# alexkeroro86/SampleNeRFRO

Hardware: AMD Instinct MI355X
Metric: rays/sec (train step) (higher is better)
Workload: dtype f16x3/fp32-acc

## Files before the change

include/rnerf.h:

```cpp
#ifndef RNERF_H_
#define RNERF_H_

#include <stddef.h>
#include <stdint.h>

#ifdef __cplusplus
extern "C" {
#endif

#define RNERF_VERSION 4

enum rnerf_status {
  RNERF_OK = 0,
  RNERF_ERR_ARG = -1,
  RNERF_ERR_HIP = -2,
  RNERF_ERR_UNSUPPORTED = -3
};

enum rnerf_precision {
  RNERF_PREC_F32 = 0,
  RNERF_PREC_F16X3 = 1,
  RNERF_PREC_BF16X3 = 2,
  RNERF_PREC_F16 = 3,
  RNERF_PREC_BF16 = 4,
// ... 178 lines not shown
  int32_t bg_patch_size;
  double bg_weight, bg_smooth_weight, annealed_alpha;
  double frozen_sq;
  int64_t frozen_count;
  void* aux_stream;
  void* grads_stream;
} rnerf_train_cfg;
typedef struct rnerf_prefetch {
  const float* origins;
  const float* viewdirs;
  float* path_pd;
  float* path_dr;
  void* side_stream;
} rnerf_prefetch;
size_t rnerf_train_workspace_bytes(const rnerf_model* m, const rnerf_train_cfg* c, int32_t B);
int rnerf_train_forward_backward(const rnerf_model* m, const rnerf_train_cfg* c, const float* theta, const float* origins, const float* viewdirs,
                                 const float* pixels, const float* env_dirs, int32_t B, const uint32_t* keys4, const int32_t* jitter_override,
                                 const float* u_override, int32_t u_per_ray, const float* path_pd, const float* path_dr, float* grads,
                                 void* workspace, int32_t max_workgroups, const rnerf_prefetch* next, void* stream);

#define RNERF_ADAM_SCRATCH_FLOATS 3076
typedef struct rnerf_adam_cfg {
  double lr_init, lr_final, lr_delay_mult;
  int64_t max_steps, lr_delay_steps;
  double b1, b2, eps;
  double weight_decay_mult, grad_max_val, grad_max_norm;
  int64_t n_all;
  double lr_override;
  int32_t use_lr_override;
  int32_t skip_nonfinite;
} rnerf_adam_cfg;
int rnerf_adam_update(const rnerf_adam_cfg* c, float* theta, float* mu, float* nu, float* grads, int64_t n_theta, const float* frozen_params,
                      int64_t n_frozen, int32_t* step_counter, float* scratch, void* stream);

int rnerf_graph_begin(void* stream);
int rnerf_graph_end(void* stream, void** graph_exec);
int rnerf_graph_launch(void* graph_exec, void* stream);
int rnerf_graph_destroy(void* graph_exec);
int rnerf_fork(void* main_stream, void* side_stream);
int rnerf_join(void* main_stream, void* side_stream);

size_t rnerf_ssim_workspace_bytes(int64_t n, int32_t H, int32_t W, int32_t C, int32_t filter_size);
int rnerf_ssim(const float* img0, const float* img1, int64_t n, int32_t H, int32_t W, int32_t C, int32_t filter_size, double filter_sigma,
               double max_val, double k1, double k2, float* map, float* mean, void* workspace, void* stream);

#ifdef __cplusplus
}
#endif
#endif
```

samplenerfro_amd/_lib.py:

```python
from __future__ import annotations

import ctypes as C
import os
from typing import Optional

HERE = os.path.dirname(os.path.abspath(__file__))
LIB_PATH = os.path.join(HERE, "lib", "librnerf.so")

PREC_F32, PREC_F16X3, PREC_BF16X3, PREC_F16, PREC_BF16, PREC_F16X2, PREC_F16F8 = 0, 1, 2, 3, 4, 5, 6
PRECISIONS = {"f32": PREC_F32, "f16x3": PREC_F16X3, "bf16x3": PREC_BF16X3, "f16": PREC_F16, "bf16": PREC_BF16, "f16x2": PREC_F16X2, "f16f8": PREC_F16F8}
BWD_BF16, BWD_F16, BWD_F16X2 = 0, 1, 2
BWD_F16X3 = BWD_F16X2
BWD_F16X3_LO8 = 4
BACKWARDS = {"f16x3": BWD_F16X3, "f16x3lo8": BWD_F16X3_LO8, "f16": BWD_F16, "bf16": BWD_BF16, "f32": BWD_F16X3, "tf32": BWD_F16}
BACKWARD_NAMES = {BWD_F16X3: "f16x3", BWD_F16X3_LO8: "f16x3lo8", BWD_F16: "f16", BWD_BF16: "bf16"}
TWO_PLANE_BACKWARDS = (BWD_F16X3, BWD_F16X3_LO8)
ABI_VERSION = 4
NERFMLP_PARAMS = 595844
BKGDMLP_PARAMS = 56963
SO3MLP_PARAMS = 65411


class RnerfError(RuntimeError):
    pass
# ... 75 lines not shown
    "rnerf_nerfmlp_wgrad": (C.c_int, [C.c_int, C.c_int, _vp, _vp, _i64, _vp, _vp, _vp]),
    "rnerf_voxelize": (C.c_int, [_vp, _vp, _vp, _vp, _i32, _vp, _GP, _i32, _dbl, _dbl, _vp, _vp, _vp, _vp]),
    "rnerf_voxelize_samples": (C.c_int, [_vp, _vp, _vp, _vp, _i32, _vp, _GP, _i32, _vp, _vp, _vp]),
    "rnerf_voxelize_majority": (C.c_int, [_vp, _vp, _vp, _i32, _i32, _dbl, _dbl, _vp, _vp, _vp]),
    "rnerf_so3_query": (C.c_int, [_vp, _GP, _vp, _vp, _vp, _vp, _i64, _vp, _vp, _vp]),
    "rnerf_march_all": (C.c_int, [_vp, _GP, _vp, _vp, _vp, _vp, _vp, _i32, _dbl, _dbl, _i32, _vp, _vp, _vp, _vp, _vp]),
    "rnerf_generate_rays": (C.c_int, [_vp, _i32, _dbl, _dbl, _dbl, _dbl, _dbl, _i32, _i32, _i32, _vp, _vp, _vp, _vp]),
    "rnerf_sample_batch": (C.c_int, [_vp, _i32, _i32, _dbl, _dbl, _dbl, _dbl, _dbl, _i32, _i32, _vp, _i32, _vp, _i32, _vp, _vp, _vp, _vp, _vp, _vp]),
    "rnerf_stratified_u": (C.c_int, [_vp, _i32, _i32, _vp, _vp]),
    "rnerf_bkgd_save_bytes": (C.c_size_t, [_i64]),
    "rnerf_bkgd_dy_bytes": (C.c_size_t, [_i64]),
    "rnerf_bkgd_forward_train": (C.c_int, [_vp, _vp, _i32, _i64, _dbl, _vp, _vp, _vp]),
    "rnerf_bkgd_backward": (C.c_int, [_vp, _vp, _vp, _i64, _dbl, _vp, _vp, _vp, _vp]),
    "rnerf_theta_sumsq": (C.c_int, [_vp, _i64, _vp, _vp]),
    "rnerf_march_all_train": (C.c_int, [_vp, _GP, _vp, _vp, _vp, _vp, _vp, _i32, _dbl, _dbl, _i32, _vp, _vp, _vp, _vp, _i32, _vp, _vp, _vp, _vp, _vp, _vp]),
    "rnerf_so3_packed_bytes": (C.c_size_t, []),
    "rnerf_so3_save_bytes": (C.c_size_t, [_i64]),
    "rnerf_so3_dy_bytes": (C.c_size_t, [_i64]),
    "rnerf_so3_forward_train": (C.c_int, [_vp, _vp, _vp, _i64, _vp, _vp]),
    "rnerf_so3_backward": (C.c_int, [_vp, _vp, _vp, _vp, _i64, _vp, _i64, _vp, _vp, _vp, _vp]),
    "rnerf_so3_pair_jacobian": (C.c_int, [_vp, _GP, _vp, _vp, _vp, _vp, _i64, _vp, _vp, _vp]),
    "rnerf_march_adjoint": (C.c_int, [_vp, _GP, _vp, _vp, _vp, _vp, _vp, _vp, _vp, _vp, _i32, _dbl, _dbl, _i32, _vp, _vp]),
    "rnerf_nerfmlp_input_grad": (C.c_int, [_vp, C.c_int, _vp, _vp, _vp, _vp, _i32, _i32, _vp, _vp, _vp]),
    "rnerf_resample": (C.c_int, [_vp, _vp, _i32, _i32, _vp, _i32, _vp, _vp, _i32, _i32, _vp, _vp, _vp, _vp, _vp]),
    "rnerf_integrated_pos_enc": (C.c_int, [_vp, _vp, _vp, _i32, _i32, _vp, _dbl, _i32, _i32, _vp, _vp, _vp, _vp]),
    "rnerf_rng_split3": (C.c_int, [_vp, _vp, _vp]),
    "rnerf_rng_forward": (C.c_int, [_vp, _i32, _i32, _i32, _vp, _vp, _vp]),
    "rnerf_stratified_u_dev": (C.c_int, [_vp, _i32, _i32, _vp, _vp]),
    "rnerf_forward_workspace_bytes": (C.c_size_t, [_MP, _i32]),
    "rnerf_forward": (C.c_int, [_MP, _vp, _vp, _i32, _vp, _vp, _i32, _vp, _vp, _vp, _vp, _vp, _i32, _vp]),
    "rnerf_train_workspace_bytes": (C.c_size_t, [_MP, _TP, _i32]),
    "rnerf_train_forward_backward": (C.c_int, [_MP, _TP, _vp, _vp, _vp, _vp, _vp, _i32, _vp, _vp, _vp, _i32, _vp, _vp, _vp, _vp, _i32, C.POINTER(Prefetch), _vp]),
    "rnerf_adam_update": (C.c_int, [_AP, _vp, _vp, _vp, _vp, _i64, _vp, _i64, _vp, _vp, _vp]),
    "rnerf_graph_begin": (C.c_int, [_vp]),
    "rnerf_graph_end": (C.c_int, [_vp, C.POINTER(C.c_void_p)]),
    "rnerf_graph_launch": (C.c_int, [_vp, _vp]),
    "rnerf_graph_destroy": (C.c_int, [_vp]),
    "rnerf_fork": (C.c_int, [_vp, _vp]),
    "rnerf_join": (C.c_int, [_vp, _vp]),
    "rnerf_ssim_workspace_bytes": (C.c_size_t, [_i64, _i32, _i32, _i32, _i32]),
    "rnerf_ssim": (C.c_int, [_vp, _vp, _i64, _i32, _i32, _i32, _i32, _dbl, _dbl, _dbl, _dbl, _vp, _vp, _vp, _vp]),
}

_lib: Optional[C.CDLL] = None


def load(path: Optional[str] = None) -> C.CDLL:
    global _lib
    if _lib is not None and path is None:
        return _lib
    p = path or LIB_PATH
    if not os.path.exists(p):
        raise RnerfError(f"{p} not found: build it with `python -m samplenerfro_amd.build` "
                         "(there is no CPU fallback for the hot path)")
    lib = C.CDLL(p)
    for name, (res, args) in SIGNATURES.items():
        fn = getattr(lib, name)
        fn.restype = res
        fn.argtypes = args
    got = lib.rnerf_version()
    if got != ABI_VERSION:
        raise RnerfError(f"{p} speaks ABI version {got}, this binding was written for {ABI_VERSION} (include/rnerf.h RNERF_VERSION): rebuild with "
                         "`python -m samplenerfro_amd.build --force`")
    if path is None or _lib is None:
        _lib = lib
    return lib
# ... 18 lines not shown
```

samplenerfro_amd/csrc/pipeline.hip:

```cpp
#include "common.h"

#include <math.h>
#include <mutex>
#include <utility>
#include <vector>

namespace rnerf {
static int current_device_cus() {
  static int cache[64] = {0};
  int dev = 0;
  if (hipGetDevice(&dev) != hipSuccess || dev < 0 || dev >= 64) return 256;
  if (cache[dev] == 0) {
    int cus = 0;
    cache[dev] = (hipDeviceGetAttribute(&cus, hipDeviceAttributeMultiprocessorCount, dev) == hipSuccess && cus > 0) ? cus : 256;
  }
  return cache[dev];
}

namespace {
constexpr size_t kPoolCap = 32;
struct EventPool { std::vector<hipEvent_t> free_[64]; };
thread_local EventPool tl_pool;
inline hipError_t pool_get(hipEvent_t* e) {
  int dev = 0;
// ... 94 lines not shown
    u[(size_t)f * B + b] = fminf(fadd(fmul((float)f, s), r), one_m_eps);
  };
  put(j, x0);
  if (j + half < size) put(j + half, x1);
}

__global__ void linspace_u_kernel(int F, double stop, float* __restrict__ u) {
  const int i = blockIdx.x * blockDim.x + threadIdx.x;
  if (i >= F) return;
  const double step = F > 1 ? stop / (double)(F - 1) : 0.0;
  u[i] = (F > 1 && i == F - 1) ? (float)stop : (float)((double)i * step);
}

__global__ void __launch_bounds__(256) bkgd_dirs_kernel(const float4* __restrict__ path_dr, const int* __restrict__ jitter, int Nc, int B,
                                                        const float* __restrict__ env, int M, float4* __restrict__ dst) {
  const int i = blockIdx.x * blockDim.x + threadIdx.x;
  if (i < B) {
    const float4 d = path_dr[(size_t)jitter[Nc - 1] * B + i];
    dst[i] = make_float4(d.x, d.y, d.z, 0.f);
  } else if (i < B + M) {
    const int e = i - B;
    dst[i] = make_float4(env[3 * e], env[3 * e + 1], env[3 * e + 2], 0.f);
  }
}

__global__ void __launch_bounds__(256) bd_cut_mul_kernel(const float* __restrict__ trans, const float* __restrict__ behind, int B,
                                                         float* __restrict__ out) {
  const int i = blockIdx.x * blockDim.x + threadIdx.x;
  if (i < 3 * B) out[i] = fmul(trans[i / 3], behind[i]);
}

constexpr int ADAM_BLOCKS = 1024;
__global__ void __launch_bounds__(256) adam_prep_kernel(const float* __restrict__ theta, float* __restrict__ g, long long n, float wd2, float max_val,
                                                        int want_norm, float* __restrict__ partial, float* __restrict__ bad_partial) {
  float s = 0.f;
  int bad = 0;
  for (long long i = (long long)blockIdx.x * blockDim.x + threadIdx.x; i < n; i += (long long)gridDim.x * blockDim.x) {
    float v = g[i];
    if (wd2 != 0.f) v = v + theta[i] * wd2;
    const bool nf = !(fabsf(v) <= 3.402823466e38f);
    bad += nf;
    if (max_val > 0.f && !nf) v = fminf(fmaxf(v, -max_val), max_val);
    g[i] = v;
    s += v * v;
  }
  __shared__ float red[4];
  __shared__ int redb[4];
  for (int o = 32; o > 0; o >>= 1) { s += __shfl_down(s, o); bad += __shfl_down(bad, o); }
  if ((threadIdx.x & 63) == 0) { red[threadIdx.x >> 6] = s; redb[threadIdx.x >> 6] = bad; }
  __syncthreads();
  if (threadIdx.x == 0) {
    if (want_norm) partial[blockIdx.x] = (red[0] + red[1]) + (red[2] + red[3]);
    bad_partial[blockIdx.x] = (float)((redb[0] + redb[1]) + (redb[2] + redb[3]));
  }
}
__global__ void __launch_bounds__(256) adam_frozen_sq_kernel(const float* __restrict__ frozen, long long n, float wd2, float max_val,
                                                             float* __restrict__ partial) {
  float s = 0.f;
  for (long long i = (long long)blockIdx.x * blockDim.x + threadIdx.x; i < n; i += (long long)gridDim.x * blockDim.x) {
    float v = frozen[i] * wd2;
    if (max_val > 0.f) v = fminf(fmaxf(v, -max_val), max_val);
    s += v * v;
  }
  __shared__ float red[4];
  for (int o = 32; o > 0; o >>= 1) s += __shfl_down(s, o);
  if ((threadIdx.x & 63) == 0) red[threadIdx.x >> 6] = s;
  __syncthreads();
  if (threadIdx.x == 0) partial[blockIdx.x] = (red[0] + red[1]) + (red[2] + red[3]);
}
struct AdamSched { double lr_init, lr_final, lr_delay_mult, max_steps, lr_delay_steps, b1, b2, max_norm, lr_override; int use_override, skip_nonfinite; };
__global__ void __launch_bounds__(256) adam_scalars_kernel(AdamSched c, int* __restrict__ step, const float* __restrict__ partial, int n_partial,
                                                           const float* __restrict__ bad_partial, float* __restrict__ scal) {
  __shared__ double red[256];
  double s = 0.0;
  for (int i = threadIdx.x; i < n_partial; i += 256) s += (double)partial[i];
  red[threadIdx.x] = s;
  __syncthreads();
  for (int o = 128; o > 0; o >>= 1) { if ((int)threadIdx.x < o) red[threadIdx.x] += red[threadIdx.x + o]; __syncthreads(); }
  const double sumsq = red[0];
  __syncthreads();
  double nb = 0.0;
  if (bad_partial) for (int i = threadIdx.x; i < ADAM_BLOCKS; i += 256) nb += (double)bad_partial[i];
  red[threadIdx.x] = nb;
  __syncthreads();
  for (int o = 128; o > 0; o >>= 1) { if ((int)threadIdx.x < o) red[threadIdx.x] += red[threadIdx.x + o]; __syncthreads(); }
  if (threadIdx.x != 0) return;
  const int count = *step;
  const double t = (double)count + 1.0;
  double lr;
  if (c.use_override) {
    lr = c.lr_override;
  } else {
    double delay = 1.0;
    if (c.lr_delay_steps > 0) {
      const double x = fmin(fmax((double)count / c.lr_delay_steps, 0.0), 1.0);
      delay = c.lr_delay_mult + (1.0 - c.lr_delay_mult) * sin(0.5 * 3.141592653589793 * x);
    }
    const double start = fmin(fmax((double)count, 0.0), 1.0);
    const double tt = fmin(fmax(fmax((double)count, 0.0) / c.max_steps, 0.0), 1.0);
    lr = start * delay * exp(log(c.lr_init) * (1.0 - tt) + log(c.lr_final) * tt);
  }
  const double bad = red[0];
  scal[0] = (float)(-lr / (1.0 - pow(c.b1, t)));
  scal[1] = (c.skip_nonfinite && bad > 0.0) ? -1.0f : (float)(1.0 / (1.0 - pow(c.b2, t)));
  float mult = 1.0f;
  if (c.max_norm > 0) {
    const float norm = sqrtf((float)sumsq);
    mult = fminf((float)c.max_norm / (1e-7f + norm), 1.0f);
  }
  scal[2] = mult;
  scal[3] = (float)bad;
  *step = count + 1;
}
__global__ void __launch_bounds__(256) adam_apply_kernel(float* __restrict__ theta, float* __restrict__ mu, float* __restrict__ nu,
                                                         const float* __restrict__ g, long long n, float b1, float b2, float eps,
                                                         float* __restrict__ scal, int count_bad) {
  const float a = scal[0], c2 = scal[1], mult = scal[2];
  if (c2 < 0.f) return;
  int bad = 0;
  for (long long i = (long long)blockIdx.x * blockDim.x + threadIdx.x; i < n; i += (long long)gridDim.x * blockDim.x) {
    const float gi = g[i] * mult;
    bad += !(fabsf(gi) <= 3.402823466e38f);
    const float m = mu[i] * b1 + gi * (1.0f - b1);
    const float v = nu[i] * b2 + (gi * gi) * (1.0f - b2);
    mu[i] = m; nu[i] = v;
    theta[i] = theta[i] + a * (m / (sqrtf(v * c2) + eps));
  }
  if (count_bad && __builtin_amdgcn_ballot_w64(bad != 0) != 0) {
    for (int o = 32; o > 0; o >>= 1) bad += __shfl_down(bad, o);
    if ((threadIdx.x & 63) == 0 && bad) atomicAdd(&scal[3], (float)bad);
  }
}

struct Carver {
  char* base; size_t off;
  explicit Carver(void* b) : base((char*)b), off(0) {}
  template <typename T> T* take(size_t count) {
    off = (off + 255) & ~(size_t)255;
    T* p = (T*)(base ? base + off : nullptr);
    off += count * sizeof(T);
    return p;
  }
  void* bytes(size_t n) { return (void*)take<char>(n); }
};

struct FwdBuffers {
  float *path_pd, *path_dr, *bk_dirs, *bkgd, *raw_c, *weights, *u, *rows_pd, *rows_dr, *scratch, *raw_f, *tmp_level, *tmp_level2;
};
static size_t carve_forward(const rnerf_model* m, int32_t B, bool own_path, void* ws, FwdBuffers* f) {
  Carver c(ws);
  const size_t Nc = m->num_coarse, Nf = m->num_fine, N = Nc * (size_t)m->num_path, S = Nc + Nf;
  f->path_pd = own_path ? c.take<float>(N * B * 4) : nullptr;
  f->path_dr = own_path ? c.take<float>(N * B * 4) : nullptr;
  f->bk_dirs = c.take<float>((size_t)B * 4);
  f->bkgd = c.take<float>((size_t)B * 3);
  f->raw_c = c.take<float>(Nc * B * 4);
  f->weights = c.take<float>(Nc * B);
  f->u = f->rows_pd = f->rows_dr = f->scratch = f->raw_f = f->tmp_level = f->tmp_level2 = nullptr;
  if (Nf > 0) {
    f->u = c.take<float>(Nf * (size_t)B);
    f->rows_pd = c.take<float>(S * B * 4);
    f->rows_dr = c.take<float>(S * B * 4);
    f->scratch = c.take<float>(S * B);
// ... 300 lines not shown
  float* d_first = t.d_all;
  const bool split_levels = levels_side_by_side(m, c, B);
  float* d_raw_c = split_levels ? t.d_raw_c : t.d_raw;
  void* dy_c = split_levels ? t.dy_c : t.dy;
  if (Nf > 0) {
    RNERF_TRY(rnerf_composite_backward(f.raw_f, f.rows_pd, f.rows_dr, nullptr, S, B, bkgd, m->rgb_padding, m->sigma_bias, lf.rgb, pixels, lf.trans, lf.tb, t.sums,
                                       mse_scale, c->bg_weight * bg_on, t.d_raw, d_first, 0, m->white_bkgd, m->bd_cut == 1 ? 1 : level_mask_mode(m), m->bd_cut ? m->bd_cut_bbox : nullptr, stream));
    if (split_levels) {
      RNERF_TRY(rnerf_composite_backward(f.raw_c, path_pd, path_dr, jitter, Nc, B, bkgd, m->rgb_padding, m->sigma_bias, lc.rgb, pixels, nullptr, nullptr, nullptr,
                                         mse_scale, 0.0, d_raw_c, d_first, 1, m->white_bkgd, level_mask_mode(m), level_mask_box(m), stream));
      RNERF_TRY(rnerf_fork(stream, aux));
      if (smooth) RNERF_TRY(rnerf_env_smooth_backward(rgb_env, ps, c->bg_smooth_weight * env_on, t.d_all + (size_t)3 * B, t.env_sum, aux));
      RNERF_TRY(rnerf_bkgd_backward(th_b, t.save_bk, t.d_all, (int64_t)B + M, m->rgb_padding, t.dy_bk, g_b, nullptr, aux));
      RNERF_TRY(nerfmlp_dgrad_impl(t.packed_bwd, t.packed_c, prec, bwd, t.save_c, d_raw_c, (int64_t)Nc * B, dy_c, !pre_zeroed, false, (hipStream_t)aux));
      RNERF_TRY(rnerf_nerfmlp_wgrad(prec, bwd, t.save_c, dy_c, (int64_t)Nc * B, g_c, t.wgrad_ws_c, aux));
    }
    if (!aux) RNERF_TRY(rnerf_nerfmlp_pack_bwd(th_f, bwd, t.packed_bwd_f, stream));
    RNERF_TRY(nerfmlp_dgrad_impl(t.packed_bwd_f, t.packed_f, prec, bwd, t.save_f, t.d_raw, (int64_t)S * B, t.dy, !pre_zeroed, !split_levels, st));
    if (next) RNERF_TRY(march_next());
    RNERF_TRY(rnerf_nerfmlp_wgrad(prec, bwd, t.save_f, t.dy, (int64_t)S * B, g_f, t.wgrad_ws, stream));
    if (split_levels)
      RNERF_TRY(rnerf_join(stream, aux));
    else
      RNERF_TRY(rnerf_composite_backward(f.raw_c, path_pd, path_dr, jitter, Nc, B, bkgd, m->rgb_padding, m->sigma_bias, lc.rgb, pixels, nullptr, nullptr, nullptr,
                                         mse_scale, 0.0, t.d_raw, d_first, 1, m->white_bkgd, level_mask_mode(m), level_mask_box(m), stream));
  } else {
    RNERF_TRY(rnerf_composite_backward(f.raw_c, path_pd, path_dr, jitter, Nc, B, bkgd, m->rgb_padding, m->sigma_bias, lf.rgb, pixels, lf.trans, lf.tb, t.sums,
                                       mse_scale, c->bg_weight * bg_on, t.d_raw, d_first, 0, m->white_bkgd, level_mask_mode(m), level_mask_box(m), stream));
  }
  if (!aux) RNERF_TRY(rnerf_nerfmlp_pack_bwd(th_c, bwd, t.packed_bwd, stream));
  if (!split_levels)
    RNERF_TRY(nerfmlp_dgrad_impl(t.packed_bwd, t.packed_c, prec, bwd, t.save_c, t.d_raw, (int64_t)Nc * B, t.dy, !(pre_zeroed && Nf == 0), true, st));
  if (next && Nf == 0) RNERF_TRY(march_next());
  if (!split_levels) RNERF_TRY(rnerf_nerfmlp_wgrad(prec, bwd, t.save_c, t.dy, (int64_t)Nc * B, g_c, t.wgrad_ws, stream));
  if (c->grads_stream) RNERF_TRY(rnerf_fork(stream, c->grads_stream));
  if (!split_levels) {
    if (smooth) RNERF_TRY(rnerf_env_smooth_backward(rgb_env, ps, c->bg_smooth_weight * env_on, t.d_all + (size_t)3 * B, t.env_sum, stream));
    RNERF_TRY(rnerf_bkgd_backward(th_b, t.save_bk, t.d_all, (int64_t)B + M, m->rgb_padding, t.dy_bk, g_b, nullptr, stream));
  }
  RNERF_TRY(rnerf_train_stats(t.sums, B, Nf > 0, c->bg_weight * bg_on, smooth ? t.env_sum : nullptr, ps, env_on, aux ? nullptr : theta, n_theta, c->frozen_sq,
                              n_theta + c->frozen_count, stats8, stream));
  return RNERF_OK;
}

extern "C" int rnerf_adam_update(const rnerf_adam_cfg* c, float* theta, float* mu, float* nu, float* grads, int64_t n_theta, const float* frozen_params,
                                 int64_t n_frozen, int32_t* step_counter, float* scratch, void* stream) {
  RNERF_CHECK_ARG(c && theta && mu && nu && grads && step_counter && scratch, "rnerf_adam_update: null pointer");
  RNERF_CHECK_ARG(n_theta >= 1 && c->n_all >= n_theta, "rnerf_adam_update: need n_theta >= 1 and n_all >= n_theta");
  hipStream_t st = (hipStream_t)stream;
  const double wd2 = c->weight_decay_mult > 0 ? 2.0 * c->weight_decay_mult / (double)c->n_all : 0.0;
  const int want_norm = c->grad_max_norm > 0;
  float* scal = scratch;
  float* partial = scratch + 4;
  float* bad_partial = nullptr;
  int n_partial = 0;
  if (wd2 != 0.0 || c->grad_max_val > 0 || want_norm || c->skip_nonfinite) {
    bad_partial = scratch + 4 + 2 * ADAM_BLOCKS;
    hipLaunchKernelGGL(adam_prep_kernel, dim3(ADAM_BLOCKS), dim3(256), 0, st, (const float*)theta, grads, (long long)n_theta, (float)wd2, (float)c->grad_max_val,
                       want_norm, partial, bad_partial);
    if (want_norm) {
      n_partial = ADAM_BLOCKS;
      if (frozen_params && n_frozen > 0 && wd2 != 0.0) {
        hipLaunchKernelGGL(adam_frozen_sq_kernel, dim3(ADAM_BLOCKS), dim3(256), 0, st, frozen_params, (long long)n_frozen, (float)wd2, (float)c->grad_max_val,
                           partial + ADAM_BLOCKS);
        n_partial = 2 * ADAM_BLOCKS;
      }
    }
  }
  AdamSched s{c->lr_init, c->lr_final, c->lr_delay_mult, (double)c->max_steps, (double)c->lr_delay_steps, c->b1, c->b2, c->grad_max_norm, c->lr_override, c->use_lr_override != 0,
              c->skip_nonfinite != 0};
  hipLaunchKernelGGL(adam_scalars_kernel, dim3(1), dim3(256), 0, st, s, step_counter, (const float*)partial, n_partial, (const float*)bad_partial, scal);
  hipLaunchKernelGGL(adam_apply_kernel, dim3(ADAM_BLOCKS), dim3(256), 0, st, theta, mu, nu, (const float*)grads, (long long)n_theta, (float)c->b1, (float)c->b2,
                     (float)c->eps, scal, bad_partial == nullptr);
  RNERF_CHECK_LAUNCH();
  return RNERF_OK;
}

namespace {
std::mutex g_ev_mu;
thread_local std::vector<hipEvent_t> tl_capture_events;
std::vector<std::pair<void*, std::vector<hipEvent_t>>> g_graph_events;
void drop_events(std::vector<hipEvent_t>& v) {
  for (hipEvent_t e : v) (void)hipEventDestroy(e);
  v.clear();
}
}

extern "C" int rnerf_graph_begin(void* stream) {
  drop_events(tl_capture_events);
  RNERF_CHECK_HIP(hipStreamBeginCapture((hipStream_t)stream, hipStreamCaptureModeThreadLocal));
  return RNERF_OK;
}

extern "C" int rnerf_graph_end(void* stream, void** graph_exec) {
  RNERF_CHECK_ARG(graph_exec, "rnerf_graph_end: null pointer");
  hipGraph_t g = nullptr;
  hipError_t err = hipStreamEndCapture((hipStream_t)stream, &g);
  if (err != hipSuccess) { drop_events(tl_capture_events); set_error("hipStreamEndCapture failed: %s", hipGetErrorString(err)); return RNERF_ERR_HIP; }
  hipGraphExec_t e = nullptr;
  err = hipGraphInstantiate(&e, g, nullptr, nullptr, 0);
  hipGraphDestroy(g);
  if (err != hipSuccess) { drop_events(tl_capture_events); set_error("hipGraphInstantiate failed: %s", hipGetErrorString(err)); return RNERF_ERR_HIP; }
  {
    std::lock_guard<std::mutex> l(g_ev_mu);
    g_graph_events.emplace_back((void*)e, std::move(tl_capture_events));
  }
  tl_capture_events.clear();
  *graph_exec = (void*)e;
// ... 60 lines not shown
```

samplenerfro_amd/graph.py:

```python
from __future__ import annotations

import ctypes as C
import os
from typing import Any, Dict, Optional

import numpy as np
import torch

from . import _lib, distributed, ops
from .train import TrainState, _bump, adam_cfg, frozen_sq_of, train_cfg
from .utils import Rays, Stats


class GraphTrainStep:
    def __init__(self, model, state: TrainState, flags, batch_size: int, rng, env_rays: Optional[Rays] = None, annealed_alpha: float = 0.5,
                 prefetch: bool = True):
        if not flags.stage.startswith("radiance"):
            raise NotImplementedError("GraphTrainStep: the radiance stages (stage all* reads a device counter back every step)")
        if state._lr_fn_default is not state.lr_fn:
            raise ValueError("GraphTrainStep evaluates the reference's learning-rate schedule on the device; state.lr_fn was replaced")
        self.lib = _lib.load()
        self.model, self.state, self.flags = model, state, flags
        self.B = int(batch_size)
        dev = state.theta.device
# ... 59 lines not shown
        k = 1 - self.slot if self.prefetch else self.slot
        return {"origins": self.origins[k], "viewdirs": self.viewdirs[k], "pixels": self.pixels[k]}

    def order_after_loader(self) -> None:
        self.main.wait_stream(torch.cuda.current_stream())

    def _march(self, slot: int, stream) -> None:
        k = slot if self.prefetch else 0
        m = self.model
        _lib.check(self.lib.rnerf_march(m.table.data_ptr(), C.byref(m.spec), self.origins[slot].data_ptr(), self.viewdirs[slot].data_ptr(), self.B,
                                        m.near, m.far, m.num_samples, self.path_pd[k].data_ptr(), self.path_dr[k].data_ptr(), None, None, stream),
                   "rnerf_march")

    def _issue_front(self, slot: int) -> None:
        lib, st, sd = self.lib, self.main.cuda_stream, self.side.cuda_stream
        k = slot if self.prefetch else 0
        _lib.check(lib.rnerf_rng_split3(self.rng_state.data_ptr(), self.keys4.data_ptr(), st), "rnerf_rng_split3")
        if not self.prefetch:
            self._march(slot, st)
        nxt = None
        if self.prefetch:
            nxt = _lib.Prefetch(self.origins[1 - slot].data_ptr(), self.viewdirs[1 - slot].data_ptr(), self.path_pd[1 - slot].data_ptr(),
                                self.path_dr[1 - slot].data_ptr(), sd)
        _lib.check(lib.rnerf_train_forward_backward(C.byref(self.m), C.byref(self.c), self.state.theta.data_ptr(), self.origins[slot].data_ptr(),
                                                    self.viewdirs[slot].data_ptr(), self.pixels[slot].data_ptr(), _lib.ptr(self.env), self.B,
                                                    self.keys4.data_ptr(), None, None, 0, self.path_pd[k].data_ptr(), self.path_dr[k].data_ptr(),
                                                    self.state.grads.data_ptr(), self.ws.data_ptr(), 0, C.byref(nxt) if nxt is not None else None, st),
                   "rnerf_train_forward_backward")

    def _issue_back(self) -> None:
        s = self.state
        fs = frozen_sq_of(s, s.variables)
        frozen = s.variables["flat"].get("so3_mlp") if fs[1] > 0 else None
        _lib.check(self.lib.rnerf_adam_update(C.byref(self.a), s.theta.data_ptr(), s.mu.data_ptr(), s.nu.data_ptr(), s.grads.data_ptr(), s.theta.numel(),
                                              _lib.ptr(frozen), fs[1], s.step_dev.data_ptr(), s.adam_scratch.data_ptr(), self.main.cuda_stream),
                   "rnerf_adam_update")

    def _capture(self, slot: int):
        lib, st, sd = self.lib, self.main.cuda_stream, self.side.cuda_stream
        out = C.c_void_p()
        if not self.split:
            _lib.check(lib.rnerf_graph_begin(st), "rnerf_graph_begin")
            self._issue_front(slot)
            self._issue_back()
            if self.prefetch:
                _lib.check(lib.rnerf_join(st, sd), "rnerf_join")
            _lib.check(lib.rnerf_graph_end(st, C.byref(out)), "rnerf_graph_end")
            return (out.value, None)
        _lib.check(lib.rnerf_graph_begin(st), "rnerf_graph_begin")
        self._issue_front(slot)
        if self.prefetch:
            _lib.check(lib.rnerf_join(st, sd), "rnerf_join")
        _lib.check(lib.rnerf_graph_end(st, C.byref(out)), "rnerf_graph_end")
        back = C.c_void_p()
        _lib.check(lib.rnerf_graph_begin(st), "rnerf_graph_begin")
        self._issue_back()
        _lib.check(lib.rnerf_graph_end(st, C.byref(back)), "rnerf_graph_end")
        return (out.value, back.value)

    def _warm(self, slot: int) -> None:
        self._issue_front(slot)
        if self.prefetch:
            _lib.check(self.lib.rnerf_join(self.main.cuda_stream, self.side.cuda_stream), "rnerf_join")
        if self.split:
            with torch.cuda.stream(self.main):
                distributed.allreduce_mean_([self.state.grads])
        self._issue_back()

    def step(self, annealed_alpha: Optional[float] = None) -> Stats:
# ... 58 lines not shown
```

samplenerfro_amd/train.py:

```python
from __future__ import annotations

import contextlib
import ctypes as C
import os
import weakref
from typing import Any, Dict, Optional

import numpy as np
import torch

from . import _lib, distributed, ops, prng
from .models import BKGD_MLP_SHAPES, NERF_MLP_SHAPES, SO3_MLP_SHAPES, NerfModel, make_variables
from .utils import Rays, Stats, learning_rate_decay

_RANGE_RETRY_LAG = 2
_LAG_SLOTS = 8
_SKIP_NONFINITE_UPDATES = True

_N_STATS = 8


class TrainState:

    def __init__(self, step, theta, mu, nu, variables, segments, lr_fn, flags=None):
        self.step, self.theta, self.mu, self.nu = step, theta, mu, nu
        self.flags = flags
        self.variables, self.segments, self.lr_fn = variables, segments, lr_fn
        self.grads = torch.zeros(theta.numel() + _N_STATS, dtype=torch.float32, device=theta.device)
        self.frozen_sq: Optional[torch.Tensor] = None
        self.next_path = None
        self._lr_fn_default = lr_fn
        self.step_dev = torch.zeros(1, dtype=torch.int32, device=theta.device) if theta.is_cuda else None
        self._step_dev_value = 0
        self.adam_scratch = torch.zeros(_lib.ADAM_SCRATCH_FLOATS, dtype=torch.float32, device=theta.device) if theta.is_cuda else None
        self._staged_bad: Optional[int] = None
        self.range_retries = 0
        self.range_retry_failures = 0
        self._model_ref = None
        self._lag_pending = []
        self._lag_host = torch.zeros(_LAG_SLOTS, dtype=torch.float32).pin_memory() if theta.is_cuda else None
        self._lag_count = 0
        self.last_retry_stats = None

    def nonfinite_grads(self) -> int:
        if self._staged_bad is not None:
            return self._staged_bad
        return int(self.adam_scratch[3].item()) if self.adam_scratch is not None else 0

    def sync_step_counter(self) -> None:
        if self.step_dev is not None and self._step_dev_value != self.step:
            self.step_dev.fill_(int(self.step))
            self._step_dev_value = self.step

    @classmethod
    def create(cls, model: NerfModel, variables: Dict[str, Any], flags) -> "TrainState":
        names = ["coarse_mlp"] + (["fine_mlp"] if model.num_fine_samples > 0 else []) + ["bkgd_mlp"]
        stage = getattr(flags, "stage", "radiance")
        if stage.startswith("all"):
            names.append("so3_mlp")
        elif stage.startswith("ior"):
            names = ["so3_mlp"]
        shapes = {"coarse_mlp": NERF_MLP_SHAPES, "fine_mlp": NERF_MLP_SHAPES, "bkgd_mlp": BKGD_MLP_SHAPES, "so3_mlp": SO3_MLP_SHAPES}
        parts = [model._flat(variables, n, shapes[n]).detach().reshape(-1).float() for n in names]
        theta = torch.cat(parts).contiguous()
        segments, off = {}, 0
        flat = dict(variables.get("flat", {}))
        for n, p in zip(names, parts):
            segments[n] = (off, off + p.numel())
            flat[n] = theta[off:off + p.numel()]
            off += p.numel()
        new_vars = make_variables(flat)
        lr_fn = lambda count: learning_rate_decay(count, flags.lr_init, flags.lr_final, flags.max_steps, flags.lr_delay_steps,
                                                  flags.lr_delay_mult)
        return cls(0, theta, torch.zeros_like(theta), torch.zeros_like(theta), new_vars, segments, lr_fn, flags)
# ... 137 lines not shown

def train_cfg(model: NerfModel, state: TrainState, flags, annealed: float) -> "_lib.TrainCfg":
    c = _lib.TrainCfg()
    c.backward = backward_mode(flags, model)
    c.randomized, c.use_random_choice = int(bool(flags.randomized)), int(model.use_random_choice)
    c.bg_patch_size = int(flags.bg_patch_size) if flags.bg_smooth_weight > 0 else 0
    c.bg_weight, c.bg_smooth_weight, c.annealed_alpha = float(flags.bg_weight), float(flags.bg_smooth_weight), float(annealed)
    fs = frozen_sq_of(state, state.variables)
    c.frozen_sq, c.frozen_count = fs[0], fs[1]
    c.aux_stream = model.tail_stream().cuda_stream
    return c


def adam_cfg(state: TrainState, flags, lr_override: Optional[float] = None) -> "_lib.AdamCfg":
    a = _lib.AdamCfg()
    a.lr_init, a.lr_final, a.lr_delay_mult = float(flags.lr_init), float(flags.lr_final), float(flags.lr_delay_mult)
    a.max_steps, a.lr_delay_steps = int(flags.max_steps), int(flags.lr_delay_steps)
    a.b1, a.b2, a.eps = 0.9, 0.999, 1e-8
    a.weight_decay_mult, a.grad_max_val, a.grad_max_norm = float(flags.weight_decay_mult), float(flags.grad_max_val), float(flags.grad_max_norm)
    a.n_all = state.theta.numel() + frozen_sq_of(state, state.variables)[1]
    a.use_lr_override = int(lr_override is not None)
    a.lr_override = float(lr_override) if lr_override is not None else 0.0
    a.skip_nonfinite = int(_SKIP_NONFINITE_UPDATES)
    return a


def _adam_update_on_device(state: TrainState, flags) -> None:
    lib = _lib.load()
    default_lr = state._lr_fn_default is state.lr_fn
    a = adam_cfg(state, flags, None if default_lr else float(state.lr_fn(state.step)))
    state.sync_step_counter()
    fs = frozen_sq_of(state, state.variables)
    frozen = state.variables["flat"].get("so3_mlp") if fs[1] > 0 else None
    _lib.check(lib.rnerf_adam_update(C.byref(a), state.theta.data_ptr(), state.mu.data_ptr(), state.nu.data_ptr(), state.grads.data_ptr(), state.theta.numel(),
                                     _lib.ptr(frozen), fs[1], state.step_dev.data_ptr(), state.adam_scratch.data_ptr(), _lib.current_stream()), "rnerf_adam_update")
    state.step += 1
    state._step_dev_value = state.step
    state._staged_bad = None
    _bump(state.theta)


def _train_step_whole(model: NerfModel, rng, state: TrainState, batch, flags, jitter, u_fine, path, next_rays):
    lib = _lib.load()
    rng, key_0, key_1 = prng.split(np.asarray(rng, np.uint32), 3)
    annealed = float(np.asarray(batch["annealed_alpha"]).reshape(-1)[0])
    rays: Rays = batch["rays"]
    o, v = ops._chk(rays.origins, "origins"), ops._chk(rays.viewdirs, "viewdirs")
    pixels = ops._chk(batch["pixels"][..., :3].contiguous(), "pixels")
    B = o.shape[0]
    env = None
    if flags.bg_smooth_weight > 0:
        env = ops._chk(batch["env_rays"].viewdirs.reshape(-1, 3), "env_rays.viewdirs")
        if env.shape[0] != flags.bg_patch_size ** 2:
            raise ValueError("env_rays.viewdirs must hold bg_patch_size^2 directions")
    m = model.c_model()
    c = train_cfg(model, state, flags, annealed)
    st = _lib.current_stream()
    keys = model._keys_dev(key_0, key_1)
    jit = model._jitter_dev(jitter) if jitter is not None else None
    u, per_ray = None, 0
    if u_fine is not None:
        u = ops._chk(u_fine, "u_fine"); per_ray = 1 if u.dim() == 2 else 0
    pd = dr = None
    if path is not None:
        if path.batch != B:
            raise ValueError("path handle was marched for a different batch size")
        cur = torch.cuda.current_stream()
        cur.wait_event(path.event)
# ... 32 lines not shown
    return state, stats, rng


def _bump(t: torch.Tensor) -> None:
    try:
        torch._C._autograd._unsafe_set_version_counter([t], [t._version + 1])
    except (AttributeError, TypeError):
        t.add_(0)


@contextlib.contextmanager
def range_safe(model: NerfModel, flags):
    saved = (model.precision, model._packed, getattr(flags, "backward_precision", "f16x3"))
    model.precision, model._packed, flags.backward_precision = _lib.PREC_BF16X3, {}, "bf16"
    try:
        yield model
    finally:
        model.precision, model._packed, flags.backward_precision = saved


_F16_BASED = (_lib.PREC_F16X3, _lib.PREC_F16)


def train_step(model: NerfModel, rng, state: TrainState, batch: Dict[str, Any], flags=None, *, range_retry=None, **kw):
    flags = state.flags if flags is None else flags
    mode = getattr(flags, "range_retry", False) if range_retry is None else range_retry
    retry = bool(mode)
    if not (retry and flags.stage.startswith("radiance") and model.precision in _F16_BASED):
        return _train_step_once(model, rng, state, batch, flags, **kw)
    if mode == "lag":
        if kw.get("taps") is not None or kw.get("forward_taps") is not None or torch.cuda.is_current_stream_capturing():
            return _train_step_once(model, rng, state, batch, flags, **kw)
        ctx = _dist_context()
        out = _train_step_once(model, rng, state, batch, flags, **kw)
        slot = state._lag_count % _LAG_SLOTS
        state._lag_count += 1
        state._lag_host[slot:slot + 1].copy_(state.adam_scratch[3:4], non_blocking=True)
        ev = torch.cuda.Event(); ev.record()
        replay = dict(kw, next_rays=None, path=None)
        state._lag_pending.append((ev, slot, rng, _clone_batch(batch), flags, replay, ctx))
        state._model_ref = weakref.ref(model)
        while len(state._lag_pending) > _RANGE_RETRY_LAG:
            pend = state._lag_pending.pop(0)
            if _lag_flag(state, pend):
                out = (out[0], _clone_stats(out[1]), out[2])
            _settle_lagged(model, state, pend)
        return out
    step0 = state.step
    out = _train_step_once(model, rng, state, batch, flags, _guard=True, **kw)
    if state.nonfinite_grads() == 0:
        return out
    next_path = state.next_path
    state.step = step0
    state.sync_step_counter()
    kw = dict(kw, next_rays=None)
    with range_safe(model, flags):
        out = _train_step_once(model, rng, state, batch, flags, _guard=True, **kw)
    state.next_path = next_path
    _count_rerun(state)
    return out


def _dist_context():
    return (distributed._GROUP, bool(distributed._skip()))


@contextlib.contextmanager
def _in_dist_context(ctx):
    saved = (distributed._GROUP, distributed._SKIP)
    distributed._GROUP, distributed._SKIP = ctx
# ... 217 lines not shown
```

Baseline: 639,500.

## Fuse Adam scalar computation into apply kernel and overlap backward tail on aux stream

Merges the single-block Adam scalar kernel into the apply kernel, with each block recomputing the schedule scalars, and moves the step-counter increment into the prep kernel, removing one launch and a serial single-block stage. The background/env-smooth backward and stats kernels move to the aux stream to overlap with the NeRF MLP weight-gradient kernel. The nonfinite count can be written directly to pinned host memory instead of via a separate async copy. Risks include redundant per-block reductions and extra stream fork/join overhead.

After: 650,800, median of 6. 1.8% higher.

```diff
diff --git a/include/rnerf.h b/include/rnerf.h
--- a/include/rnerf.h
+++ b/include/rnerf.h
@@ -234,6 +234,9 @@
 } rnerf_adam_cfg;
 int rnerf_adam_update(const rnerf_adam_cfg* c, float* theta, float* mu, float* nu, float* grads, int64_t n_theta, const float* frozen_params,
                       int64_t n_frozen, int32_t* step_counter, float* scratch, void* stream);
+int rnerf_adam_update_fused(const rnerf_adam_cfg* c, float* theta, float* mu, float* nu, float* grads, int64_t n_theta,
+                            const float* frozen_params, int64_t n_frozen, int32_t* step_counter, float* scratch, float* nonfinite_out,
+                            void* stream);
 
 int rnerf_graph_begin(void* stream);
 int rnerf_graph_end(void* stream, void** graph_exec);
diff --git a/samplenerfro_amd/_lib.py b/samplenerfro_amd/_lib.py
--- a/samplenerfro_amd/_lib.py
+++ b/samplenerfro_amd/_lib.py
@@ -131,6 +131,7 @@
     "rnerf_train_workspace_bytes": (C.c_size_t, [_MP, _TP, _i32]),
     "rnerf_train_forward_backward": (C.c_int, [_MP, _TP, _vp, _vp, _vp, _vp, _vp, _i32, _vp, _vp, _vp, _i32, _vp, _vp, _vp, _vp, _i32, C.POINTER(Prefetch), _vp]),
     "rnerf_adam_update": (C.c_int, [_AP, _vp, _vp, _vp, _vp, _i64, _vp, _i64, _vp, _vp, _vp]),
+    "rnerf_adam_update_fused": (C.c_int, [_AP, _vp, _vp, _vp, _vp, _i64, _vp, _i64, _vp, _vp, _vp, _vp]),
     "rnerf_graph_begin": (C.c_int, [_vp]),
     "rnerf_graph_end": (C.c_int, [_vp, C.POINTER(C.c_void_p)]),
     "rnerf_graph_launch": (C.c_int, [_vp, _vp]),
diff --git a/samplenerfro_amd/csrc/pipeline.hip b/samplenerfro_amd/csrc/pipeline.hip
--- a/samplenerfro_amd/csrc/pipeline.hip
+++ b/samplenerfro_amd/csrc/pipeline.hip
@@ -150,7 +150,8 @@
 
 constexpr int ADAM_BLOCKS = 1024;
 __global__ void __launch_bounds__(256) adam_prep_kernel(const float* __restrict__ theta, float* __restrict__ g, long long n, float wd2, float max_val,
-                                                        int want_norm, float* __restrict__ partial, float* __restrict__ bad_partial) {
+                                                        int want_norm, float* __restrict__ partial, float* __restrict__ bad_partial,
+                                                        int* __restrict__ step_inc) {
   float s = 0.f;
   int bad = 0;
   for (long long i = (long long)blockIdx.x * blockDim.x + threadIdx.x; i < n; i += (long long)gridDim.x * blockDim.x) {
@@ -170,6 +171,7 @@
   if (threadIdx.x == 0) {
     if (want_norm) partial[blockIdx.x] = (red[0] + red[1]) + (red[2] + red[3]);
     bad_partial[blockIdx.x] = (float)((redb[0] + redb[1]) + (redb[2] + redb[3]));
+    if (step_inc && blockIdx.x == 0) *step_inc = *step_inc + 1;
   }
 }
 __global__ void __launch_bounds__(256) adam_frozen_sq_kernel(const float* __restrict__ frozen, long long n, float wd2, float max_val,
@@ -187,9 +189,8 @@
   if (threadIdx.x == 0) partial[blockIdx.x] = (red[0] + red[1]) + (red[2] + red[3]);
 }
 struct AdamSched { double lr_init, lr_final, lr_delay_mult, max_steps, lr_delay_steps, b1, b2, max_norm, lr_override; int use_override, skip_nonfinite; };
-__global__ void __launch_bounds__(256) adam_scalars_kernel(AdamSched c, int* __restrict__ step, const float* __restrict__ partial, int n_partial,
-                                                           const float* __restrict__ bad_partial, float* __restrict__ scal) {
-  __shared__ double red[256];
+__device__ __forceinline__ void adam_scalars_block(const AdamSched& c, int count, const float* __restrict__ partial, int n_partial,
+                                                   const float* __restrict__ bad_partial, double* red, float* out) {
   double s = 0.0;
   for (int i = threadIdx.x; i < n_partial; i += 256) s += (double)partial[i];
   red[threadIdx.x] = s;
@@ -203,7 +204,6 @@
   __syncthreads();
   for (int o = 128; o > 0; o >>= 1) { if ((int)threadIdx.x < o) red[threadIdx.x] += red[threadIdx.x + o]; __syncthreads(); }
   if (threadIdx.x != 0) return;
-  const int count = *step;
   const double t = (double)count + 1.0;
   double lr;
   if (c.use_override) {
@@ -219,16 +219,22 @@
     lr = start * delay * exp(log(c.lr_init) * (1.0 - tt) + log(c.lr_final) * tt);
   }
   const double bad = red[0];
-  scal[0] = (float)(-lr / (1.0 - pow(c.b1, t)));
-  scal[1] = (c.skip_nonfinite && bad > 0.0) ? -1.0f : (float)(1.0 / (1.0 - pow(c.b2, t)));
+  out[0] = (float)(-lr / (1.0 - pow(c.b1, t)));
+  out[1] = (c.skip_nonfinite && bad > 0.0) ? -1.0f : (float)(1.0 / (1.0 - pow(c.b2, t)));
   float mult = 1.0f;
   if (c.max_norm > 0) {
     const float norm = sqrtf((float)sumsq);
     mult = fminf((float)c.max_norm / (1e-7f + norm), 1.0f);
   }
-  scal[2] = mult;
-  scal[3] = (float)bad;
-  *step = count + 1;
+  out[2] = mult;
+  out[3] = (float)bad;
+}
+__global__ void __launch_bounds__(256) adam_scalars_kernel(AdamSched c, int* __restrict__ step, const float* __restrict__ partial, int n_partial,
+                                                           const float* __restrict__ bad_partial, float* __restrict__ scal) {
+  __shared__ double red[256];
+  const int count = *step;
+  adam_scalars_block(c, count, partial, n_partial, bad_partial, red, scal);
+  if (threadIdx.x == 0) *step = count + 1;
 }
 __global__ void __launch_bounds__(256) adam_apply_kernel(float* __restrict__ theta, float* __restrict__ mu, float* __restrict__ nu,
                                                          const float* __restrict__ g, long long n, float b1, float b2, float eps,
@@ -247,6 +253,30 @@
   if (count_bad && __builtin_amdgcn_ballot_w64(bad != 0) != 0) {
     for (int o = 32; o > 0; o >>= 1) bad += __shfl_down(bad, o);
     if ((threadIdx.x & 63) == 0 && bad) atomicAdd(&scal[3], (float)bad);
+  }
+}
+
+__global__ void __launch_bounds__(256) adam_apply_fused_kernel(AdamSched c, const int* __restrict__ step, const float* __restrict__ partial,
+                                                               int n_partial, const float* __restrict__ bad_partial, float* __restrict__ theta,
+                                                               float* __restrict__ mu, float* __restrict__ nu, const float* __restrict__ g,
+                                                               long long n, float b1, float b2, float eps, float* __restrict__ scal,
+                                                               float* __restrict__ count_out) {
+  __shared__ double red[256];
+  __shared__ float sc[4];
+  adam_scalars_block(c, *step - 1, partial, n_partial, bad_partial, red, sc);
+  __syncthreads();
+  const float a = sc[0], c2 = sc[1], mult = sc[2];
+  if (blockIdx.x == 0 && threadIdx.x == 0) {
+    scal[0] = a; scal[1] = c2; scal[2] = mult; scal[3] = sc[3];
+    if (count_out) *count_out = sc[3];
+  }
+  if (c2 < 0.f) return;
+  for (long long i = (long long)blockIdx.x * blockDim.x + threadIdx.x; i < n; i += (long long)gridDim.x * blockDim.x) {
+    const float gi = g[i] * mult;
+    const float m = mu[i] * b1 + gi * (1.0f - b1);
+    const float v = nu[i] * b2 + (gi * gi) * (1.0f - b2);
+    mu[i] = m; nu[i] = v;
+    theta[i] = theta[i] + a * (m / (sqrtf(v * c2) + eps));
   }
 }
 
@@ -613,22 +643,27 @@
   if (!split_levels)
     RNERF_TRY(nerfmlp_dgrad_impl(t.packed_bwd, t.packed_c, prec, bwd, t.save_c, t.d_raw, (int64_t)Nc * B, t.dy, !(pre_zeroed && Nf == 0), true, st));
   if (next && Nf == 0) RNERF_TRY(march_next());
-  if (!split_levels) RNERF_TRY(rnerf_nerfmlp_wgrad(prec, bwd, t.save_c, t.dy, (int64_t)Nc * B, g_c, t.wgrad_ws, stream));
-  if (c->grads_stream) RNERF_TRY(rnerf_fork(stream, c->grads_stream));
+  const bool tail_on_aux = aux && !split_levels;
+  void* tail = tail_on_aux ? aux : stream;
+  if (tail_on_aux) RNERF_TRY(rnerf_fork(stream, aux));
+  if (!split_levels && !tail_on_aux) RNERF_TRY(rnerf_nerfmlp_wgrad(prec, bwd, t.save_c, t.dy, (int64_t)Nc * B, g_c, t.wgrad_ws, stream));
+  if (!tail_on_aux && c->grads_stream) RNERF_TRY(rnerf_fork(stream, c->grads_stream));
   if (!split_levels) {
-    if (smooth) RNERF_TRY(rnerf_env_smooth_backward(rgb_env, ps, c->bg_smooth_weight * env_on, t.d_all + (size_t)3 * B, t.env_sum, stream));
-    RNERF_TRY(rnerf_bkgd_backward(th_b, t.save_bk, t.d_all, (int64_t)B + M, m->rgb_padding, t.dy_bk, g_b, nullptr, stream));
+    if (smooth) RNERF_TRY(rnerf_env_smooth_backward(rgb_env, ps, c->bg_smooth_weight * env_on, t.d_all + (size_t)3 * B, t.env_sum, tail));
+    RNERF_TRY(rnerf_bkgd_backward(th_b, t.save_bk, t.d_all, (int64_t)B + M, m->rgb_padding, t.dy_bk, g_b, nullptr, tail));
   }
   RNERF_TRY(rnerf_train_stats(t.sums, B, Nf > 0, c->bg_weight * bg_on, smooth ? t.env_sum : nullptr, ps, env_on, aux ? nullptr : theta, n_theta, c->frozen_sq,
-                              n_theta + c->frozen_count, stats8, stream));
-  return RNERF_OK;
-}
-
-extern "C" int rnerf_adam_update(const rnerf_adam_cfg* c, float* theta, float* mu, float* nu, float* grads, int64_t n_theta, const float* frozen_params,
-                                 int64_t n_frozen, int32_t* step_counter, float* scratch, void* stream) {
-  RNERF_CHECK_ARG(c && theta && mu && nu && grads && step_counter && scratch, "rnerf_adam_update: null pointer");
-  RNERF_CHECK_ARG(n_theta >= 1 && c->n_all >= n_theta, "rnerf_adam_update: need n_theta >= 1 and n_all >= n_theta");
-  hipStream_t st = (hipStream_t)stream;
+                              n_theta + c->frozen_count, stats8, tail));
+  if (tail_on_aux) {
+    RNERF_TRY(rnerf_nerfmlp_wgrad(prec, bwd, t.save_c, t.dy, (int64_t)Nc * B, g_c, t.wgrad_ws, stream));
+    if (c->grads_stream) RNERF_TRY(rnerf_fork(stream, c->grads_stream));
+    RNERF_TRY(rnerf_join(stream, aux));
+  }
+  return RNERF_OK;
+}
+
+static int adam_update_impl(const rnerf_adam_cfg* c, float* theta, float* mu, float* nu, float* grads, int64_t n_theta, const float* frozen_params,
+                            int64_t n_frozen, int32_t* step_counter, float* scratch, bool fused, float* count_out, hipStream_t st) {
   const double wd2 = c->weight_decay_mult > 0 ? 2.0 * c->weight_decay_mult / (double)c->n_all : 0.0;
   const int want_norm = c->grad_max_norm > 0;
   float* scal = scratch;
@@ -638,7 +673,7 @@
   if (wd2 != 0.0 || c->grad_max_val > 0 || want_norm || c->skip_nonfinite) {
     bad_partial = scratch + 4 + 2 * ADAM_BLOCKS;
     hipLaunchKernelGGL(adam_prep_kernel, dim3(ADAM_BLOCKS), dim3(256), 0, st, (const float*)theta, grads, (long long)n_theta, (float)wd2, (float)c->grad_max_val,
-                       want_norm, partial, bad_partial);
+                       want_norm, partial, bad_partial, fused ? step_counter : nullptr);
     if (want_norm) {
       n_partial = ADAM_BLOCKS;
       if (frozen_params && n_frozen > 0 && wd2 != 0.0) {
@@ -650,11 +685,32 @@
   }
   AdamSched s{c->lr_init, c->lr_final, c->lr_delay_mult, (double)c->max_steps, (double)c->lr_delay_steps, c->b1, c->b2, c->grad_max_norm, c->lr_override, c->use_lr_override != 0,
               c->skip_nonfinite != 0};
+  if (fused && bad_partial) {
+    hipLaunchKernelGGL(adam_apply_fused_kernel, dim3(ADAM_BLOCKS), dim3(256), 0, st, s, (const int*)step_counter, (const float*)partial, n_partial,
+                       (const float*)bad_partial, theta, mu, nu, (const float*)grads, (long long)n_theta, (float)c->b1, (float)c->b2, (float)c->eps, scal, count_out);
+    RNERF_CHECK_LAUNCH();
+    return RNERF_OK;
+  }
   hipLaunchKernelGGL(adam_scalars_kernel, dim3(1), dim3(256), 0, st, s, step_counter, (const float*)partial, n_partial, (const float*)bad_partial, scal);
   hipLaunchKernelGGL(adam_apply_kernel, dim3(ADAM_BLOCKS), dim3(256), 0, st, theta, mu, nu, (const float*)grads, (long long)n_theta, (float)c->b1, (float)c->b2,
                      (float)c->eps, scal, bad_partial == nullptr);
   RNERF_CHECK_LAUNCH();
-  return RNERF_OK;
+  if (count_out) RNERF_CHECK_HIP(hipMemcpyAsync(count_out, scal + 3, sizeof(float), hipMemcpyDefault, st));
+  return RNERF_OK;
+}
+
+extern "C" int rnerf_adam_update(const rnerf_adam_cfg* c, float* theta, float* mu, float* nu, float* grads, int64_t n_theta, const float* frozen_params,
+                                 int64_t n_frozen, int32_t* step_counter, float* scratch, void* stream) {
+  RNERF_CHECK_ARG(c && theta && mu && nu && grads && step_counter && scratch, "rnerf_adam_update: null pointer");
+  RNERF_CHECK_ARG(n_theta >= 1 && c->n_all >= n_theta, "rnerf_adam_update: need n_theta >= 1 and n_all >= n_theta");
+  return adam_update_impl(c, theta, mu, nu, grads, n_theta, frozen_params, n_frozen, step_counter, scratch, false, nullptr, (hipStream_t)stream);
+}
+
+extern "C" int rnerf_adam_update_fused(const rnerf_adam_cfg* c, float* theta, float* mu, float* nu, float* grads, int64_t n_theta, const float* frozen_params,
+                                       int64_t n_frozen, int32_t* step_counter, float* scratch, float* nonfinite_out, void* stream) {
+  RNERF_CHECK_ARG(c && theta && mu && nu && grads && step_counter && scratch, "rnerf_adam_update_fused: null pointer");
+  RNERF_CHECK_ARG(n_theta >= 1 && c->n_all >= n_theta, "rnerf_adam_update_fused: need n_theta >= 1 and n_all >= n_theta");
+  return adam_update_impl(c, theta, mu, nu, grads, n_theta, frozen_params, n_frozen, step_counter, scratch, true, nonfinite_out, (hipStream_t)stream);
 }
 
 namespace {
diff --git a/samplenerfro_amd/graph.py b/samplenerfro_amd/graph.py
--- a/samplenerfro_amd/graph.py
+++ b/samplenerfro_amd/graph.py
@@ -115,9 +115,9 @@
         s = self.state
         fs = frozen_sq_of(s, s.variables)
         frozen = s.variables["flat"].get("so3_mlp") if fs[1] > 0 else None
-        _lib.check(self.lib.rnerf_adam_update(C.byref(self.a), s.theta.data_ptr(), s.mu.data_ptr(), s.nu.data_ptr(), s.grads.data_ptr(), s.theta.numel(),
-                                              _lib.ptr(frozen), fs[1], s.step_dev.data_ptr(), s.adam_scratch.data_ptr(), self.main.cuda_stream),
-                   "rnerf_adam_update")
+        _lib.check(self.lib.rnerf_adam_update_fused(C.byref(self.a), s.theta.data_ptr(), s.mu.data_ptr(), s.nu.data_ptr(), s.grads.data_ptr(), s.theta.numel(),
+                                                    _lib.ptr(frozen), fs[1], s.step_dev.data_ptr(), s.adam_scratch.data_ptr(), None, self.main.cuda_stream),
+                   "rnerf_adam_update_fused")
 
     def _capture(self, slot: int):
         lib, st, sd = self.lib, self.main.cuda_stream, self.side.cuda_stream
diff --git a/samplenerfro_amd/train.py b/samplenerfro_amd/train.py
--- a/samplenerfro_amd/train.py
+++ b/samplenerfro_amd/train.py
@@ -40,6 +40,8 @@
         self._lag_pending = []
         self._lag_host = torch.zeros(_LAG_SLOTS, dtype=torch.float32).pin_memory() if theta.is_cuda else None
         self._lag_count = 0
+        self._lag_word = None
+        self._lag_word_written = False
         self.last_retry_stats = None
 
     def nonfinite_grads(self) -> int:
@@ -243,8 +245,12 @@
     state.sync_step_counter()
     fs = frozen_sq_of(state, state.variables)
     frozen = state.variables["flat"].get("so3_mlp") if fs[1] > 0 else None
-    _lib.check(lib.rnerf_adam_update(C.byref(a), state.theta.data_ptr(), state.mu.data_ptr(), state.nu.data_ptr(), state.grads.data_ptr(), state.theta.numel(),
-                                     _lib.ptr(frozen), fs[1], state.step_dev.data_ptr(), state.adam_scratch.data_ptr(), _lib.current_stream()), "rnerf_adam_update")
+    word = getattr(state, "_lag_word", None)
+    _lib.check(lib.rnerf_adam_update_fused(C.byref(a), state.theta.data_ptr(), state.mu.data_ptr(), state.nu.data_ptr(), state.grads.data_ptr(),
+                                           state.theta.numel(), _lib.ptr(frozen), fs[1], state.step_dev.data_ptr(), state.adam_scratch.data_ptr(),
+                                           word, _lib.current_stream()), "rnerf_adam_update_fused")
+    if word is not None:
+        state._lag_word_written = True
     state.step += 1
     state._step_dev_value = state.step
     state._staged_bad = None
@@ -343,10 +349,15 @@
         if kw.get("taps") is not None or kw.get("forward_taps") is not None or torch.cuda.is_current_stream_capturing():
             return _train_step_once(model, rng, state, batch, flags, **kw)
         ctx = _dist_context()
-        out = _train_step_once(model, rng, state, batch, flags, **kw)
         slot = state._lag_count % _LAG_SLOTS
         state._lag_count += 1
-        state._lag_host[slot:slot + 1].copy_(state.adam_scratch[3:4], non_blocking=True)
+        state._lag_word, state._lag_word_written = state._lag_host[slot:slot + 1].data_ptr(), False
+        try:
+            out = _train_step_once(model, rng, state, batch, flags, **kw)
+        finally:
+            state._lag_word = None
+        if not state._lag_word_written:
+            state._lag_host[slot:slot + 1].copy_(state.adam_scratch[3:4], non_blocking=True)
         ev = torch.cuda.Event(); ev.record()
         replay = dict(kw, next_rays=None, path=None)
         state._lag_pending.append((ev, slot, rng, _clone_batch(batch), flags, replay, ctx))
```
